# grahamstockton87/RayTracingOneWeekendApplication

Hardware: NVIDIA B200
Metric: path-tracing throughput (higher is better)
Workload: dtype f32

## Files before the change

raytracingoneweekendapplication_b200/csrc/rt_b200.cu:

```cuda
#include <cuda_runtime.h>

#include <chrono>
#include <cmath>
#include <cstdarg>
#include <cstdio>
#include <cstdlib>
#include <cstring>
#include <string>
#include <thread>
#include <vector>

#include "bvh_build.h"
#include "bvh_wide.h"
#include "prim_derive.h"
#include "bvh_device.cuh"
#include "rt_b200.h"
#include "rt_device.cuh"
#include "rt_wide.cuh"
#ifdef RT_B200_ALT_KERNELS
#include "rt_wavefront.cuh"
#endif

using namespace rtdev;

struct RenderArgs {
    int width, height;
    int max_depth;
    int spp_begin;
    int n_local_samples;
    int sample_stride, sample_offset;
    int seg_len;
    int n_segments;
    int tiles_x, tiles_y, tile_size;
    int tile_stride, tile_offset;
    int n_local_tiles;
    int blocks_per_tile_x, blocks_per_tile_y;
    unsigned long long n_items;
    uint32_t k0, k1;
    int compact;
    int nee_emitters;
    int shadow_point_lights;
};

constexpr float kAccumScale = 268435456.0f;
constexpr float kSampleClamp = 1048576.0f;

#ifdef RT_B200_ALT_KERNELS
#include "rt_kernel_v1.cuh"
#endif

#ifndef RT_TRAV_THRESHOLD
#define RT_TRAV_THRESHOLD 4
#endif
#ifndef RT_B200_DEFAULT_BVH_WIDTH
#define RT_B200_DEFAULT_BVH_WIDTH 2
#endif
#ifndef RT_MIN_BLOCKS
#define RT_MIN_BLOCKS 4
#endif
#ifndef RT_WIDE_MIN_BLOCKS
#define RT_WIDE_MIN_BLOCKS RT_MIN_BLOCKS
#endif
#ifndef RT_V2_THREADS
#define RT_V2_THREADS 256
#endif
constexpr int kTravHistBins = 208;
constexpr int kTravThreshold = RT_TRAV_THRESHOLD;
enum : int { LANE_IDLE = 0, LANE_TRAVERSE = 1, LANE_SHADE = 2 };

template <int WIDTH>
struct TravSel { using Trav = TravW<WIDTH>; using RayConst = RayConstW; };
template <>
struct TravSel<2> { using Trav = rtdev::Trav; using RayConst = rtdev::RayConst; };

enum : int { FEAT_MEDIA = 1, FEAT_MEDIA_GENERAL = 2, FEAT_SPECULAR = 4, FEAT_MSPHERE = 8, FEAT_TRI = 16, FEAT_LIGHTS = 32,
             FEAT_DEFOCUS = 64, FEAT_ALL = 127 };
template <bool STATS, bool LITE, bool NEE = false, int WIDTH = 2, int FEAT = FEAT_ALL>
__global__ void __launch_bounds__(RT_V2_THREADS, WIDTH == 2 ? RT_MIN_BLOCKS : RT_WIDE_MIN_BLOCKS) render_kernel_v2(const __grid_constant__ DevScene S, const __grid_constant__ RenderArgs A,
                                                        unsigned long long* __restrict__ accum,
                                                        unsigned long long* __restrict__ counters, Stats* __restrict__ gstats) {
    constexpr bool NO_TRI = LITE || !(FEAT & FEAT_TRI), NO_DEFOCUS = LITE || !(FEAT & FEAT_DEFOCUS), LIGHTS = !LITE && (FEAT & FEAT_LIGHTS);
    const unsigned lane = threadIdx.x & 31u;
    const unsigned lt_mask = (1u << lane) - 1u;
    Stats st;
    if (STATS) memset(&st, 0, sizeof st);

    unsigned pool_pos = 0, pool_size = 0;
    int blk_x0 = 0, blk_y0 = 0, seg_s0 = 0;
    __shared__ uint32_t lane_slot[RT_V2_THREADS];
    unsigned slot_base = 0;
    bool exhausted = A.max_depth <= 0;

    int state = LANE_IDLE;
    Rng rng;
    rng.pixel = rng.sample = 0;
    rng.k0 = A.k0;
    rng.k1 = A.k1;
    Ray ray;
    ray.o = ray.d = v3(0, 0, 0);
    ray.time = 0;
    V3 L = v3(0, 0, 0), T = v3(1, 1, 1);
    uint32_t bounce = 0, origin_prim = PRIM_NONE;
    float nee_pdf = 0.0f;
    typename TravSel<WIDTH>::Trav tr;
    StackEntry stack_mem[WIDTH == 2 ? STACK_SIZE : 1];
    extern __shared__ uint2 wide_stack_mem[];
    auto stack = [&]() {
        if constexpr (WIDTH == 2) return &stack_mem[0];
        else return SmemStack<RT_V2_THREADS>::make(wide_stack_mem);
    }();
    tr.clear();
    tr.hit.t = 0;
    tr.hit.prim = PRIM_NONE;
    tr.hit.u = tr.hit.v = 0;
    const float kInf = __int_as_float(0x7f800000);
    unsigned seg_steps = 0, n_leaf = 0;
    unsigned long long* hist = reinterpret_cast<unsigned long long*>(gstats + 1);

    while (true) {
        unsigned needy = __ballot_sync(0xffffffffu, state == LANE_IDLE);
        while (needy && !exhausted) {
            if (pool_pos >= pool_size) {
                unsigned long long item = 0;
                if (lane == 0) item = atomicAdd(&counters[0], 1ull);
                item = __shfl_sync(0xffffffffu, item, 0);
                if (item >= A.n_items) {
                    exhausted = true;
                    break;
                }
                const unsigned seg = (unsigned)(item % (unsigned long long)A.n_segments);
                const unsigned long long blk = item / (unsigned long long)A.n_segments;
                const unsigned blocks_per_tile = (unsigned)(A.blocks_per_tile_x * A.blocks_per_tile_y);
                const unsigned local_tile = (unsigned)(blk / blocks_per_tile), in_tile = (unsigned)(blk % blocks_per_tile);
                const unsigned tile = A.tile_offset + local_tile * A.tile_stride;
                blk_x0 = (int)(tile % A.tiles_x) * A.tile_size + (int)(in_tile % A.blocks_per_tile_x) * 8;
                blk_y0 = (int)(tile / A.tiles_x) * A.tile_size + (int)(in_tile / A.blocks_per_tile_x) * 4;
                seg_s0 = (int)seg * A.seg_len;
                pool_size = 32u * (unsigned)min(A.seg_len, A.n_local_samples - seg_s0);
                pool_pos = 0;
                slot_base = (local_tile * (unsigned)A.tile_size + (in_tile / (unsigned)A.blocks_per_tile_x) * 4u) * (unsigned)A.tile_size +
                            (in_tile % (unsigned)A.blocks_per_tile_x) * 8u;
            }
            const unsigned e = pool_pos + __popc(needy & lt_mask);
            if (state == LANE_IDLE && e < pool_size) {
                const int px = blk_x0 + (int)(e & 7u), py = blk_y0 + (int)((e >> 3) & 3u);
                if (px < A.width && py < A.height) {
                    rng.pixel = (uint32_t)(py * A.width + px);
                    rng.sample = (uint32_t)(A.spp_begin + A.sample_offset + (seg_s0 + (int)(e >> 5)) * A.sample_stride);
                    if (A.compact) lane_slot[threadIdx.x] = slot_base + ((e >> 3) & 3u) * (unsigned)A.tile_size + (e & 7u);
                    ray = camera_ray<NO_DEFOCUS>(S, px, py, rng);
                    L = v3(0, 0, 0);
                    T = v3(1, 1, 1);
                    bounce = 0;
                    origin_prim = PRIM_NONE;
                    nee_pdf = 0.0f;
                    tr.init(S, kInf);
                    state = tr.done() ? LANE_SHADE : LANE_TRAVERSE;
                    if (STATS) { st.samples++; st.rays++; seg_steps = n_leaf = 0; }
                }
            }
            pool_pos += min((unsigned)__popc(needy), pool_size - pool_pos);
            needy = __ballot_sync(0xffffffffu, state == LANE_IDLE);
        }
        if (__ballot_sync(0xffffffffu, state != LANE_IDLE) == 0u) break;

        {
            typename TravSel<WIDTH>::RayConst rc;
            rc.set(ray);
            while (true) {
                while (true) {
                    const bool descending = tr.wants_node();
                    if (!STATS) {
                        if (!__any_sync(0xffffffffu, descending)) break;
                    }
                    const unsigned dmask = STATS ? __ballot_sync(0xffffffffu, descending) : 1u;
                    if (dmask == 0u) break;
                    if (STATS) {
                        const unsigned tmask = __ballot_sync(0xffffffffu, state == LANE_TRAVERSE);
                        if (lane == 0) { st.desc_iters++; st.desc_lanes += __popc(dmask); st.desc_trav_lanes += __popc(tmask); }
                    }
                    if (descending) {
                        tr.template node_step<STATS>(S, ray, rc, 0.001f, stack, &st);
                        if (STATS) {
                            seg_steps++;
                            if (tr.done()) {
                                atomicAdd(hist + 128 + min(seg_steps, 63u), 1ull);
                                atomicAdd(hist + 192 + min(n_leaf, 15u), 1ull);
                            }
                        }
                    }
                }
                if (STATS) {
                    const unsigned lmask = __ballot_sync(0xffffffffu, state == LANE_TRAVERSE && !tr.wants_node() && !tr.done());
                    if (lane == 0 && lmask) { st.leaf_iters++; st.leaf_lanes += __popc(lmask); }
                }
                if (state == LANE_TRAVERSE && !tr.wants_node()) {
                    if (!tr.done()) {
                        tr.template leaf_step<STATS, NO_TRI, (FEAT & FEAT_MSPHERE) != 0>(S, ray, rc, 0.001f, origin_prim, stack, &st);
                        if (STATS) {
                            atomicAdd(hist + (n_leaf ? 64 : 0) + min(seg_steps, 63u), 1ull);
                            n_leaf++;
                            seg_steps = 0;
                            if (tr.done()) {
                                atomicAdd(hist + 128, 1ull);
                                atomicAdd(hist + 192 + min(n_leaf, 15u), 1ull);
                            }
                        }
                    }
                    if (tr.done()) state = LANE_SHADE;
                }
                const unsigned active = __ballot_sync(0xffffffffu, state == LANE_TRAVERSE);
                if (active == 0u || __popc(active) < kTravThreshold) break;
            }
        }

        if (STATS) {
            const unsigned smask = __ballot_sync(0xffffffffu, state == LANE_SHADE);
            if (lane == 0) { st.shade_iters++; st.shade_lanes += __popc(smask); }
        }
        if (state == LANE_SHADE) {
            Hit hit = tr.hit;
            int medium = -1;
            if ((FEAT & FEAT_MEDIA) && S.n_media > 0) medium = media_hit<STATS, (FEAT & FEAT_MEDIA_GENERAL) != 0>(S, ray, 0.001f, hit.t, rng, bounce, &st);
            bool done = false;
            if (medium < 0 && hit.prim == PRIM_NONE) {
                L = L + T * v3(S.background);
                done = true;
            } else {
                Surface sf;
                if (medium >= 0) {
                    const DevMedium& md = S.media[medium];
                    sf.t = hit.t;
                    sf.p = fma3(hit.t, ray.d, ray.o);
                    sf.normal = v3(md.normal);
                    sf.front = true;
                    sf.u = sf.v = 0.0f;
                    sf.material = md.material;
                    sf.prim_id = -1;
                    sf.nee_light = 0;
                    origin_prim = PRIM_NONE;
                } else {
                    complete_hit<NO_TRI, (FEAT & FEAT_MSPHERE) != 0>(S, ray, hit, sf, false);
                    origin_prim = hit.prim;
                }
                const DevMaterial& m = S.mats[sf.material];
                float4 u4 = make_float4(0, 0, 0, 0);
                if (m.type != RT_MAT_DIFFUSE_LIGHT && m.type != RT_MAT_EMISSIVE_LIGHT) u4 = rng.draw(bounce, RS_SCATTER);
                V3 att, emitted;
                Ray next;
                const bool scattered = shade_surface<(FEAT & FEAT_SPECULAR) != 0>(S, m, ray, sf, u4, emitted, att, next);
                if (NEE && nee_pdf > 0.0f && medium < 0 && sf.nee_light > 0) {
                    const float d2 = dot(ray.d, ray.d);
                    const float cos_y = fabsf(dot(ray.d, v3(S.nee_lights[sf.nee_light - 1].n))) * rsqrtf(d2);
                    const float p_light = light_density(S, sf.t * sf.t * d2, fmaxf(cos_y, 1e-20f));
                    emitted = (nee_pdf / (nee_pdf + p_light)) * emitted;
                }
                L = L + T * emitted;
                if (!scattered) {
                    done = true;
                } else {
                    if (LIGHTS && S.n_lights > 0) {
                        if (NEE && A.shadow_point_lights) L = L + T * att * point_lighting_shadowed<WIDTH>(S, sf.p, sf.normal, origin_prim, ray.time);
                        else L = L + T * att * point_lighting(S, sf.p, sf.normal);
                    }
                    if (NEE) {
                        nee_pdf = 0.0f;
                        if (A.nee_emitters && S.n_nee_lights > 0 && (m.type == RT_MAT_LAMBERTIAN || m.type == RT_MAT_ISOTROPIC)) {
                            const bool iso = m.type == RT_MAT_ISOTROPIC;
                            nee_pdf = scatter_density(normalize(next.d), sf.normal, iso);
                            L = L + T * att * nee_direct<WIDTH>(S, sf.p, sf.normal, iso, origin_prim, ray.time, rng.draw(bounce, RS_NEE));
                        }
                    }
                    T = T * att;
                    ray = next;
                    bounce++;
                    if (bounce >= (uint32_t)A.max_depth) done = true;
                }
            }
            if (done) {
                unsigned long long* a = accum + 4ull * (A.compact ? lane_slot[threadIdx.x] : rng.pixel);
                if (isfinite(L.x) && isfinite(L.y) && isfinite(L.z)) {
                    atomicAdd(a + 0, __float2ull_rn(fminf(fmaxf(L.x, 0.0f), kSampleClamp) * kAccumScale));
                    atomicAdd(a + 1, __float2ull_rn(fminf(fmaxf(L.y, 0.0f), kSampleClamp) * kAccumScale));
                    atomicAdd(a + 2, __float2ull_rn(fminf(fmaxf(L.z, 0.0f), kSampleClamp) * kAccumScale));
                } else {
                    atomicAdd(a + 3, 1ull);
                    if (STATS) st.nonfinite++;
                }
                state = LANE_IDLE;
            } else {
                tr.init(S, kInf);
                state = tr.done() ? LANE_SHADE : LANE_TRAVERSE;
                if (STATS) { st.rays++; seg_steps = n_leaf = 0; }
            }
        }
    }
    if (STATS) {
        unsigned long long* g = reinterpret_cast<unsigned long long*>(gstats);
        const unsigned long long* l = reinterpret_cast<const unsigned long long*>(&st);
        for (unsigned i = 0; i < sizeof(Stats) / 8; i++) {
            unsigned long long v = l[i];
            for (int off = 16; off > 0; off >>= 1) v += __shfl_down_sync(0xffffffffu, v, off);
            if (lane == 0 && v) atomicAdd(g + i, v);
        }
    }
}

#ifdef RT_B200_ALT_KERNELS
#include "rt_kernel_v3.cuh"
#endif

typedef void (*RenderKernel)(const DevScene, const RenderArgs, unsigned long long*, unsigned long long*, Stats*);
struct FeatInstance {
    bool lite;
    int feat;
    RenderKernel kernel;
};
#define RT_INSTANCE(lite, feat) {lite, feat, render_kernel_v2<false, lite, false, 2, (feat)>}
static const FeatInstance kInstances[] = {
    RT_INSTANCE(true, 0),
    RT_INSTANCE(true, FEAT_MEDIA | FEAT_MSPHERE),
    RT_INSTANCE(true, FEAT_MEDIA | FEAT_MEDIA_GENERAL),
    RT_INSTANCE(false, FEAT_DEFOCUS),
    RT_INSTANCE(false, FEAT_TRI | FEAT_LIGHTS),
};
#undef RT_INSTANCE
constexpr int kNumInstances = (int)(sizeof(kInstances) / sizeof(kInstances[0]));

__device__ __forceinline__ void traverse_uploaded(const DevScene& S, const Ray& ray, float tmin, float tmax, Hit& hit) {
    if (S.wide_width == 8) traverse_sel<8>(S, ray, tmin, tmax, PRIM_NONE, hit);
    else if (S.wide_width == 4) traverse_sel<4>(S, ray, tmin, tmax, PRIM_NONE, hit);
    else traverse_sel<2>(S, ray, tmin, tmax, PRIM_NONE, hit);
}

__host__ __device__ inline void pair_node(float4* n) {
    const float4 a = n[0], b = n[1], c = n[2], e = n[3];
    n[0] = make_float4(a.x, c.x, a.y, c.y);
    n[1] = make_float4(a.z, c.z, b.x, e.x);
    n[2] = make_float4(b.y, e.y, b.z, e.z);
    n[3] = make_float4(a.w, b.w, 0.0f, 0.0f);
}
__global__ void pair_nodes_kernel(float4* __restrict__ nodes, int n) {
    const int i = blockIdx.x * blockDim.x + threadIdx.x;
    if (i < n) pair_node(nodes + 4 * (size_t)i);
}

struct CameraD {
    double center[3], dir00[3], du[3], dv[3];
};

__global__ void aov_kernel(const __grid_constant__ DevScene S, const __grid_constant__ CameraD C, int width, int height,
                           int* __restrict__ prim_id, float* __restrict__ t_out, float* __restrict__ normal, float* __restrict__ point,
                           float* __restrict__ uv) {
    int i = blockIdx.x * blockDim.x + threadIdx.x, j = blockIdx.y * blockDim.y + threadIdx.y;
    if (i >= width || j >= height) return;
    RayD rd;
    for (int k = 0; k < 3; k++) {
        rd.o[k] = C.center[k];
        rd.d[k] = C.dir00[k] + (double)i * C.du[k] + (double)j * C.dv[k];
    }
    rd.time = 0.0;
    Ray ray;
    ray.o = v3((float)rd.o[0], (float)rd.o[1], (float)rd.o[2]);
    ray.d = v3((float)rd.d[0], (float)rd.d[1], (float)rd.d[2]);
    ray.time = 0.0f;
    Hit hit;
    traverse_uploaded(S, ray, 0.001f, __int_as_float(0x7f800000), hit);
    size_t px = (size_t)j * width + i;
    Surface sf;
    sf.prim_id = -1;
    sf.p = sf.normal = v3(0, 0, 0);
    sf.u = sf.v = 0;
    float t = 0.0f;
    if (hit.prim != PRIM_NONE) {
        complete_hit_fp64(S, rd, hit, sf);
        t = sf.t;
    }
    if (prim_id) prim_id[px] = sf.prim_id;
    if (t_out) t_out[px] = t;
    if (normal) { normal[3 * px] = sf.normal.x; normal[3 * px + 1] = sf.normal.y; normal[3 * px + 2] = sf.normal.z; }
    if (point) { point[3 * px] = sf.p.x; point[3 * px + 1] = sf.p.y; point[3 * px + 2] = sf.p.z; }
    if (uv) { uv[2 * px] = sf.u; uv[2 * px + 1] = sf.v; }
}

__global__ void resolve_kernel(const unsigned long long* __restrict__ accum, int n_pixels, double inv_scale_spp,
                               float* __restrict__ rgb_linear, unsigned char* __restrict__ rgb8) {
    int px = blockIdx.x * blockDim.x + threadIdx.x;
    if (px >= n_pixels) return;
    for (int c = 0; c < 3; c++) {
        float lin = (float)((double)accum[4ull * px + c] * inv_scale_spp);
        if (rgb_linear) rgb_linear[3ull * px + c] = lin;
        if (rgb8) {
            float g = lin > 0.0f ? sqrtf(lin) : 0.0f;
            g = fminf(fmaxf(g, 0.0f), 0.999f);
            rgb8[3ull * px + c] = (unsigned char)(int)(255.999f * g);
        }
    }
}

__global__ void probe_texture_kernel(const __grid_constant__ DevScene S, int tex, int n, const float* __restrict__ uvp,
                                     float* __restrict__ rgb) {
    int i = blockIdx.x * blockDim.x + threadIdx.x;
    if (i >= n) return;
    V3 c = tex_value(S, tex, uvp[5 * i], uvp[5 * i + 1], v3(uvp + 5 * i + 2));
    rgb[3 * i] = c.x; rgb[3 * i + 1] = c.y; rgb[3 * i + 2] = c.z;
}

__global__ void probe_scatter_kernel(const __grid_constant__ DevScene S, int mat, int n, const float* __restrict__ in,
                                     const float* __restrict__ uni, float* __restrict__ out) {
    int i = blockIdx.x * blockDim.x + threadIdx.x;
    if (i >= n) return;
    const float* r = in + 16 * (size_t)i;
    Ray ray;
    ray.o = v3(r); ray.d = v3(r + 3); ray.time = r[6];
    Surface sf;
    sf.p = v3(r + 7); sf.normal = v3(r + 10); sf.front = r[13] != 0.0f; sf.u = r[14]; sf.v = r[15];
    sf.material = mat; sf.prim_id = -1;
    const DevMaterial& m = S.mats[mat];
    V3 em = mat_emitted(S, m, sf);
    float4 u4 = make_float4(uni[4 * i], uni[4 * i + 1], uni[4 * i + 2], uni[4 * i + 3]);
    V3 att = v3(0, 0, 0);
    Ray next;
    next.o = next.d = v3(0, 0, 0);
    next.time = 0;
    bool ok = mat_scatter(S, m, ray, sf, u4, att, next);
    float* o = out + 16 * (size_t)i;
    o[0] = ok ? 1.0f : 0.0f;
    o[1] = att.x; o[2] = att.y; o[3] = att.z;
    o[4] = next.o.x; o[5] = next.o.y; o[6] = next.o.z;
    o[7] = next.d.x; o[8] = next.d.y; o[9] = next.d.z;
    o[10] = em.x; o[11] = em.y; o[12] = em.z;
    o[13] = next.time; o[14] = o[15] = 0.0f;
}

__global__ void probe_hit_kernel(const __grid_constant__ DevScene S, int n, const float* __restrict__ rays, int* __restrict__ prim_id,
                                 float* __restrict__ t_out, float* __restrict__ normal, float* __restrict__ uv) {
    int i = blockIdx.x * blockDim.x + threadIdx.x;
    if (i >= n) return;
    const float* r = rays + 9 * (size_t)i;
    Ray ray;
    ray.o = v3(r); ray.d = v3(r + 3); ray.time = r[6];
    Hit hit;
    traverse_uploaded(S, ray, r[7], r[8], hit);
    Surface sf;
    sf.prim_id = -1;
    sf.normal = v3(0, 0, 0);
    sf.u = sf.v = 0;
    sf.t = 0.0f;
    if (hit.prim != PRIM_NONE) complete_hit(S, ray, hit, sf, true);
    if (prim_id) prim_id[i] = sf.prim_id;
    if (t_out) t_out[i] = sf.t;
    if (normal) { normal[3 * i] = sf.normal.x; normal[3 * i + 1] = sf.normal.y; normal[3 * i + 2] = sf.normal.z; }
    if (uv) { uv[2 * i] = sf.u; uv[2 * i + 1] = sf.v; }
}

__global__ void fma_peak_kernel(float* out, int iters, float a, float b) {
// ... 1305 lines not shown
            } else {
                rtwf::wf_extend<false><<<grid_e, 256, 0, stream>>>(ctx->scene, P, ctx->dstats);
                rtwf::wf_shade<false><<<grid_s, 256, 0, stream>>>(ctx->scene, W, P, ctx->accum, ctx->dstats);
            }
            launches += 3;
        }
        CU(ctx, cudaGetLastError());
        CU(ctx, cudaMemcpyAsync(h, P.ctr, sizeof h, cudaMemcpyDeviceToHost, stream));
        CU(ctx, cudaStreamSynchronize(stream));
        if (h[3] == 0) break;
    }
    ctx->stats.kernel_launches = launches;
    return RT_OK;
}
#endif

template <int WIDTH>
static RenderKernel v2_instance(int variant) {
    switch (variant) {
        case 1: return render_kernel_v2<false, true, false, WIDTH>;
        case 2: return render_kernel_v2<true, false, false, WIDTH>;
        default: return render_kernel_v2<false, false, false, WIDTH>;
    }
}
static int v2_effective_width(int variant, int width) { return variant >= 3 ? 2 : width; }
static RenderKernel v2_kernel(int variant, int width) {
    if (variant == 3) return render_kernel_v2<false, true, true, 2>;
    if (variant == 4) return render_kernel_v2<false, false, true, 2>;
    if (variant >= 5 && variant < 5 + kNumInstances) return kInstances[variant - 5].kernel;
    return width == 8 ? v2_instance<8>(variant) : (width == 4 ? v2_instance<4>(variant) : v2_instance<2>(variant));
}
static size_t v2_smem(const DevCtx* ctx, int width) { return width <= 2 ? 0 : (size_t)std::max(ctx->wide_depth, 1) * RT_V2_THREADS * sizeof(uint2); }

static int v2_blocks_per_sm(DevCtx* ctx, int variant, int width, int* out) {
    width = v2_effective_width(variant, width);
    RenderKernel k = v2_kernel(variant, width);
    const size_t smem = v2_smem(ctx, width);
    if (smem) {
        const int pct = (int)std::min<size_t>(100, (100 * RT_WIDE_MIN_BLOCKS * (smem + 1024) + 233471) / 233472);
        CU(ctx, cudaFuncSetAttribute((const void*)k, cudaFuncAttributePreferredSharedMemoryCarveout, pct));
    }
    CU(ctx, cudaOccupancyMaxActiveBlocksPerMultiprocessor(out, (const void*)k, RT_V2_THREADS, smem));
    return RT_OK;
}

static int launch_v2(DevCtx* ctx, int variant, int width, int grid, const RenderArgs& A, cudaStream_t stream, unsigned long long* counters = nullptr) {
    if (!counters) counters = ctx->counters;
    width = v2_effective_width(variant, width);
    v2_kernel(variant, width)<<<grid, RT_V2_THREADS, v2_smem(ctx, width), stream>>>(ctx->scene, A, ctx->accum, counters, ctx->dstats);
    return RT_OK;
}

static int dev_render(DevCtx* ctx, const rt_render_params* p) {
    if (!ctx) return RT_ERR_INVALID;
    if (!p || p->struct_size != sizeof(rt_render_params)) return fail(ctx, RT_ERR_INVALID, "rt_render: bad params struct");
    if (!ctx->has_scene) return fail(ctx, RT_ERR_STATE, "rt_render: no scene uploaded");
    if (p->width <= 0 || p->height <= 0 || p->samples_per_pixel <= 0 || p->max_depth < 0 || p->spp_begin < 0)
        return fail(ctx, RT_ERR_INVALID, "rt_render: width/height/samples must be positive");
    if ((long long)p->spp_begin + p->samples_per_pixel > 65536)
        return fail(ctx, RT_ERR_UNSUPPORTED, "rt_render: samples %d + %d exceed 65536 per pixel, the capacity of the 64-bit fixed-point sums",
                    p->spp_begin, p->samples_per_pixel);
    if ((long long)p->width * p->height >= (1ll << 31)) return fail(ctx, RT_ERR_UNSUPPORTED, "rt_render: frame too large");
    const int count = p->shard_count <= 1 ? 1 : p->shard_count;
    const int rank = count == 1 ? 0 : p->shard_rank;
    if (rank < 0 || rank >= count) return fail(ctx, RT_ERR_INVALID, "rt_render: shard_rank %d outside [0,%d)", rank, count);
    CU(ctx, cudaSetDevice(ctx->device));
    cudaStream_t stream = p->stream ? (cudaStream_t)p->stream : ctx->stream;
    const bool overlap = (p->flags & RT_FLAG_OVERLAP) && (p->flags & RT_FLAG_ASYNC) && (p->flags & RT_FLAG_ACCUMULATE) &&
                         !(p->flags & RT_FLAG_STATS) && ctx->kernel_version == 2 && ctx->accum != nullptr &&
                         ctx->cam_w == p->width && ctx->cam_h == p->height;
    int rc = overlap ? RT_OK : dev_wait(ctx);
    if (rc != RT_OK) return rc;
    if (ctx->cam_w != p->width || ctx->cam_h != p->height) setup_camera(ctx, p->width, p->height);

    RenderArgs A;
    std::memset(&A, 0, sizeof A);
    A.width = p->width;
    A.height = p->height;
    A.max_depth = p->max_depth;
    A.spp_begin = p->spp_begin;
    A.tile_size = p->tile_size > 0 ? p->tile_size : 16;
    if (A.tile_size % 8 != 0) return fail(ctx, RT_ERR_INVALID, "rt_render: tile_size must be a multiple of 8");
    A.tiles_x = (p->width + A.tile_size - 1) / A.tile_size;
    A.tiles_y = (p->height + A.tile_size - 1) / A.tile_size;
    A.blocks_per_tile_x = A.tile_size / 8;
    A.blocks_per_tile_y = A.tile_size / 4;
    const int n_tiles = A.tiles_x * A.tiles_y;
    int mode = p->shard_mode;
    if (mode == RT_SHARD_AUTO) mode = (n_tiles / count >= 256) ? RT_SHARD_TILES : RT_SHARD_SAMPLES;
    if (count == 1) mode = RT_SHARD_TILES;
    if (mode == RT_SHARD_TILES) {
        A.tile_stride = count;
        A.tile_offset = rank;
        A.n_local_tiles = (n_tiles - rank + count - 1) / count;
        A.sample_stride = 1;
        A.sample_offset = 0;
        A.n_local_samples = p->samples_per_pixel;
    } else if (mode == RT_SHARD_SAMPLES) {
        A.tile_stride = 1;
        A.tile_offset = 0;
        A.n_local_tiles = n_tiles;
        A.sample_stride = count;
        A.sample_offset = rank;
        A.n_local_samples = (p->samples_per_pixel - rank + count - 1) / count;
    } else {
        return fail(ctx, RT_ERR_INVALID, "rt_render: unknown shard_mode %d", p->shard_mode);
    }
    AccumLayout L;
    L.width = p->width;
    L.height = p->height;
    if (p->flags & RT_FLAG_COMPACT_TILES) {
        if (mode != RT_SHARD_TILES) return fail(ctx, RT_ERR_INVALID, "rt_render: RT_FLAG_COMPACT_TILES needs tile sharding (shard_mode RT_SHARD_TILES)");
        if (ctx->kernel_version != 2) return fail(ctx, RT_ERR_UNSUPPORTED, "rt_render: compact tile buffers are implemented by render_kernel_v2 only");
        L.compact = true;
        L.rank = rank;
        L.count = count;
        L.tile = A.tile_size;
        A.compact = 1;
    }
    if ((p->flags & RT_FLAG_ACCUMULATE) && ctx->accum && !(ctx->acc == L))
        return fail(ctx, RT_ERR_STATE, "rt_render: RT_FLAG_ACCUMULATE onto a buffer of another frame size or tile layout");
    rc = ensure_accum(ctx, L);
    if (rc != RT_OK) return rc;
    const bool stats = (p->flags & RT_FLAG_STATS) != 0;
    int bps = ctx->blocks_per_sm[stats ? 1 : 0];
    const bool lite = ctx->scene_lite && !getenv("RT_B200_NO_LITE");
    const bool want_nee = (p->flags & RT_FLAG_NEE) != 0 && ctx->scene.n_nee_lights > 0;
    const bool want_shadow = (p->flags & RT_FLAG_SHADOWED_POINT_LIGHTS) != 0 && ctx->scene.n_lights > 0;
    int variant = (want_nee || want_shadow) ? (lite ? 3 : 4) : (stats ? 2 : (lite ? 1 : 0));
    const int width = ctx->scene.wide_width ? ctx->scene.wide_width : 2;
    if (variant <= 1 && width == 2 && !getenv("RT_B200_GENERAL_INSTANCE"))
        for (int k = 0; k < kNumInstances; k++)
            if ((!kInstances[k].lite || lite) && (ctx->scene_feat & ~kInstances[k].feat) == 0) {
                variant = 5 + k;
                break;
            }
    if (ctx->kernel_version == 2) {
        rc = v2_blocks_per_sm(ctx, variant, width, &bps);
        if (rc != RT_OK) return rc;
    }
    const int grid = ctx->sm_count * (bps > 0 ? bps : 1);
    const unsigned long long pixel_blocks = (unsigned long long)A.n_local_tiles * A.blocks_per_tile_x * A.blocks_per_tile_y;
    const unsigned long long resident_warps = (unsigned long long)grid * (ctx->kernel_version == 2 ? RT_V2_THREADS / 32 : 8);
    int n_seg = 1;
    if (A.n_local_samples > 0 && pixel_blocks > 0) {
        unsigned long long want = (resident_warps * 64 + pixel_blocks - 1) / pixel_blocks;
        if (want < 1) want = 1;
        if (want > (unsigned long long)A.n_local_samples) want = A.n_local_samples;
        n_seg = (int)want;
    }
    A.seg_len = A.n_local_samples > 0 ? (A.n_local_samples + n_seg - 1) / n_seg : 1;
    A.n_segments = A.n_local_samples > 0 ? (A.n_local_samples + A.seg_len - 1) / A.seg_len : 0;
    A.n_items = pixel_blocks * (unsigned long long)A.n_segments;
    A.k0 = (uint32_t)(p->seed & 0xffffffffu);
    A.k1 = (uint32_t)(p->seed >> 32);

    auto pass_samples = [&]() -> uint64_t {
        if (!(mode == RT_SHARD_TILES && count > 1)) return (uint64_t)A.n_local_samples * (uint64_t)p->width * p->height;
        uint64_t px = 0;
        for (int t = rank; t < n_tiles; t += count) {
            int tx = t % A.tiles_x, ty = t / A.tiles_x;
            int w = std::min(A.tile_size, p->width - tx * A.tile_size), h = std::min(A.tile_size, p->height - ty * A.tile_size);
            px += (uint64_t)w * h;
        }
        return px * (uint64_t)A.n_local_samples;
    };
    if (overlap) {
        const int k = ctx->lane_next;
        ctx->lane_next ^= 1;
        if (!ctx->lane_stream[k]) {
            CU(ctx, cudaStreamCreateWithFlags(&ctx->lane_stream[k], cudaStreamNonBlocking));
            CU(ctx, cudaEventCreateWithFlags(&ctx->lane_end[k], cudaEventDefault));
        }
        if (!ctx->ev_fork) {
            CU(ctx, cudaEventCreateWithFlags(&ctx->ev_fork, cudaEventDisableTiming));
            CU(ctx, cudaEventCreate(&ctx->ov_begin));
        }
        cudaStream_t ls = ctx->lane_stream[k];
        unsigned long long* cnt = ctx->counters + 4 * (1 + k);
        CU(ctx, cudaEventRecord(ctx->ev_fork, stream));
        CU(ctx, cudaStreamWaitEvent(ls, ctx->ev_fork, 0));
        if (!ctx->lane_busy[0] && !ctx->lane_busy[1]) {
            CU(ctx, cudaEventRecord(ctx->ov_begin, ls));
            ctx->ov_passes = 0;
        }
        CU(ctx, cudaMemsetAsync(cnt, 0, 4 * sizeof(unsigned long long), ls));
        if (A.n_items > 0) {
            A.nee_emitters = want_nee;
            A.shadow_point_lights = want_shadow;
            rc = launch_v2(ctx, variant, width, grid, A, ls, cnt);
            if (rc != RT_OK) return rc;
            CU(ctx, cudaGetLastError());
        }
        CU(ctx, cudaEventRecord(ctx->lane_end[k], ls));
        ctx->lane_busy[k] = true;
        ctx->ov_passes++;
        ctx->stats.kernel_launches = A.n_items > 0 ? 1 : 0;
        ctx->stats.blocks = grid;
        ctx->stats.samples = pass_samples();
        return RT_OK;
    }
    if (!(p->flags & RT_FLAG_ACCUMULATE)) CU(ctx, cudaMemsetAsync(ctx->accum, 0, L.slots() * 32, stream));
    CU(ctx, cudaMemsetAsync(ctx->counters, 0, 4 * sizeof(unsigned long long), stream));
    if (stats) CU(ctx, cudaMemsetAsync(ctx->dstats, 0, sizeof(Stats) + kTravHistBins * sizeof(unsigned long long), stream));
    const bool async = (p->flags & RT_FLAG_ASYNC) != 0;
    CU(ctx, cudaEventRecord(ctx->ev0, stream));
    ctx->stats.kernel_launches = 0;
    if (A.n_items > 0) {
#ifdef RT_B200_ALT_KERNELS
        if (ctx->kernel_version == 3) {
            rc = launch_wavefront(ctx, A, stream, stats, pixel_blocks);
            if (rc != RT_OK) return rc;
        } else if (ctx->kernel_version == 1) {
            if (stats) render_kernel<true><<<grid, 256, 0, stream>>>(ctx->scene, A, ctx->accum, ctx->counters, ctx->dstats);
            else render_kernel<false><<<grid, 256, 0, stream>>>(ctx->scene, A, ctx->accum, ctx->counters, ctx->dstats);
        } else if (ctx->kernel_version == 4) {
            const bool lite = ctx->scene_lite && !getenv("RT_B200_NO_LITE");
            if (stats) render_kernel_v3<true, false><<<grid, 256, 0, stream>>>(ctx->scene, A, ctx->accum, ctx->counters, ctx->dstats);
            else if (lite) render_kernel_v3<false, true><<<grid, 256, 0, stream>>>(ctx->scene, A, ctx->accum, ctx->counters, ctx->dstats);
            else render_kernel_v3<false, false><<<grid, 256, 0, stream>>>(ctx->scene, A, ctx->accum, ctx->counters, ctx->dstats);
        } else
#endif
        {
            A.nee_emitters = want_nee;
            A.shadow_point_lights = want_shadow;
            rc = launch_v2(ctx, variant, width, grid, A, stream);
            if (rc != RT_OK) return rc;
        }
        CU(ctx, cudaGetLastError());
        if (ctx->kernel_version != 3) ctx->stats.kernel_launches = 1;
    }
    ctx->stats.blocks = grid;
    ctx->stats.samples = pass_samples();
    CU(ctx, cudaEventRecord(ctx->ev1, stream));
    ctx->pending_async = true;
    ctx->pending_stats = stats;
    ctx->pending_stream = stream;
    if (async) return RT_OK;
    return dev_wait(ctx);
}

static int dev_resolve_into(DevCtx* ctx, int32_t total_spp, float* dev_lin, unsigned char* dev_rgb8) {
    const size_t n = ctx->acc.slots();
    if (n == 0 || (!dev_lin && !dev_rgb8)) return RT_OK;
    const double inv = 1.0 / ((double)kAccumScale * (double)total_spp);
    resolve_kernel<<<(unsigned)((n + 255) / 256), 256, 0, ctx->stream>>>(ctx->accum, (int)n, inv, dev_lin, dev_rgb8);
    CU(ctx, cudaGetLastError());
    return RT_OK;
}

static int ensure_out(DevCtx* ctx, size_t pixels) {
    if (pixels <= ctx->out_pixels) return RT_OK;
    if (ctx->copy_stream) cudaStreamSynchronize(ctx->copy_stream);
    if (ctx->out_lin) cudaFree(ctx->out_lin);
    if (ctx->out_rgb8) cudaFree(ctx->out_rgb8);
    ctx->out_lin = nullptr;
    ctx->out_rgb8 = nullptr;
    ctx->out_pixels = 0;
    if (cudaMalloc(&ctx->out_lin, pixels * 3 * sizeof(float)) != cudaSuccess || cudaMalloc(&ctx->out_rgb8, pixels * 3) != cudaSuccess)
        return fail(ctx, RT_ERR_NOMEM, "rt_download: cannot allocate the output buffers");
    ctx->out_pixels = pixels;
    return RT_OK;
}

static int dev_resolve_tiles(DevCtx* ctx, int32_t total_spp, float* dev_rgb_linear, uint8_t* dev_rgb8, size_t capacity_pixels) {
    if (!ctx) return RT_ERR_INVALID;
    if (!ctx->accum) return fail(ctx, RT_ERR_STATE, "rt_resolve_tiles: nothing rendered yet");
    if (total_spp <= 0) return fail(ctx, RT_ERR_INVALID, "rt_resolve_tiles: total_spp must be positive");
    if (capacity_pixels < ctx->acc.slots()) return fail(ctx, RT_ERR_INVALID, "rt_resolve_tiles: the buffers hold %zu pixels, the frame has %zu", capacity_pixels, ctx->acc.slots());
    int rc = dev_wait(ctx);
    if (rc != RT_OK) return rc;
    rc = dev_resolve_into(ctx, total_spp, dev_rgb_linear, dev_rgb8);
    if (rc != RT_OK) return rc;
    CU(ctx, cudaStreamSynchronize(ctx->stream));
    return RT_OK;
}

static int dev_untile(DevCtx* ctx, const void* dev_shards, size_t shard_stride_bytes, int32_t bytes_per_pixel, int32_t shard_count, int32_t width,
                      int32_t height, int32_t tile_size, void* host_out) {
    if (!ctx || !dev_shards || !host_out) return RT_ERR_INVALID;
    if (width <= 0 || height <= 0 || tile_size <= 0 || shard_count <= 0 || (bytes_per_pixel != 3 && bytes_per_pixel != 12 && bytes_per_pixel != 32))
        return fail(ctx, RT_ERR_INVALID, "rt_untile: bad arguments");
    CU(ctx, cudaSetDevice(ctx->device));
    const size_t full = (size_t)width * height * bytes_per_pixel;
    int rc = ensure_scratch_out(ctx, full);
    if (rc != RT_OK) return rc;
    CU(ctx, launch_untile(bytes_per_pixel, dev_shards, shard_stride_bytes, shard_count, -1, width, height, tile_size, ctx->frame_scratch, ctx->stream));
    CU(ctx, cudaMemcpyAsync(host_out, ctx->frame_scratch, full, cudaMemcpyDeviceToHost, ctx->stream));
    CU(ctx, cudaStreamSynchronize(ctx->stream));
    return RT_OK;
}

static int frame_slot(DevCtx* ctx, size_t px, bool lin, bool rgb8, DevCtx::OutFrame** out) {
    if (ctx->frames_out >= 2) return fail(ctx, RT_ERR_STATE, "two frames are already outstanding: call rt_frame_end first");
    if (!ctx->copy_stream) CU(ctx, cudaStreamCreateWithFlags(&ctx->copy_stream, cudaStreamNonBlocking));
    if (!ctx->ev_ready) CU(ctx, cudaEventCreateWithFlags(&ctx->ev_ready, cudaEventDisableTiming));
    DevCtx::OutFrame& f = ctx->frames[ctx->frame_head];
    if (!f.done) CU(ctx, cudaEventCreateWithFlags(&f.done, cudaEventDisableTiming));
    const size_t need = (lin ? px * 12 : 0) + 256 + (rgb8 ? px * 3 : 0);
    if (need > f.cap) {
        if (f.pinned) cudaFreeHost(f.pinned);
        f.pinned = nullptr;
        f.cap = 0;
        if (cudaHostAlloc(&f.pinned, need, cudaHostAllocDefault) != cudaSuccess) return fail(ctx, RT_ERR_NOMEM, "cannot allocate %zu bytes of pinned host memory", need);
        f.cap = need;
    }
// ... 270 lines not shown
```

Before: 1855.

## Move per-warp work pool state to shared memory and use fast divisors

Per-warp work-pool bookkeeping (block origin, sample start, pool position, exhausted flag) moves from per-thread registers into a small shared-memory struct that lane 0 updates. The per-thread compact-slot shared array is dropped, and the slot is recomputed at accumulation time with precomputed multiply-shift divisors. The 64-bit div/mod in item decoding is replaced by 32-bit fast division. The aim is lower register pressure and cheaper integer work, at the cost of extra __syncwarp calls and shared-memory reads in the refill loop, plus a new limit on work items.

Measured after the change: 1879 (median of 6 runs). 1.3% higher.

```diff
diff --git a/raytracingoneweekendapplication_b200/csrc/render_args.h b/raytracingoneweekendapplication_b200/csrc/render_args.h
--- /dev/null
+++ b/raytracingoneweekendapplication_b200/csrc/render_args.h
@@ -0,0 +1,86 @@
+#pragma once
+#include <cstdint>
+
+#ifdef __CUDACC__
+#define RT_HDI __host__ __device__ __forceinline__
+#else
+#define RT_HDI inline
+#endif
+
+struct FastDiv {
+    uint32_t mul, shift;
+};
+inline FastDiv make_fast_div(uint32_t d) {
+    uint32_t l = 0;
+    while ((1ull << l) < d) l++;
+    FastDiv f;
+    f.mul = (uint32_t)(((1ull << 32) * ((1ull << l) - d)) / d + 1);
+    f.shift = l;
+    return f;
+}
+RT_HDI uint32_t fast_div(uint32_t n, FastDiv f) {
+#ifdef __CUDA_ARCH__
+    const uint32_t hi = __umulhi(n, f.mul);
+#else
+    const uint32_t hi = (uint32_t)(((uint64_t)n * f.mul) >> 32);
+#endif
+    return (hi + n) >> f.shift;
+}
+
+struct RenderArgs {
+    int width, height;
+    int max_depth;
+    int spp_begin;
+    int n_local_samples;
+    int sample_stride, sample_offset;
+    int seg_len;
+    int n_segments;
+    int tiles_x, tiles_y, tile_size;
+    int tile_stride, tile_offset;
+    int n_local_tiles;
+    int blocks_per_tile_x, blocks_per_tile_y;
+    unsigned long long n_items;
+    uint32_t k0, k1;
+    int compact;
+    int nee_emitters;
+    int shadow_point_lights;
+    FastDiv div_segments, div_tile_blocks, div_tiles_x, div_blocks_x;
+    FastDiv div_width, div_tile_size, div_tile_stride;
+};
+
+inline void set_work_divisors(RenderArgs& A) {
+    A.div_segments = make_fast_div((uint32_t)(A.n_segments > 0 ? A.n_segments : 1));
+    A.div_tile_blocks = make_fast_div((uint32_t)(A.blocks_per_tile_x * A.blocks_per_tile_y));
+    A.div_tiles_x = make_fast_div((uint32_t)A.tiles_x);
+    A.div_blocks_x = make_fast_div((uint32_t)A.blocks_per_tile_x);
+    A.div_width = make_fast_div((uint32_t)A.width);
+    A.div_tile_size = make_fast_div((uint32_t)A.tile_size);
+    A.div_tile_stride = make_fast_div((uint32_t)A.tile_stride);
+}
+
+struct PoolBlock {
+    int x0, y0, s0;
+    uint32_t size;
+};
+RT_HDI PoolBlock pool_block(const RenderArgs& A, uint32_t item) {
+    const uint32_t blk = fast_div(item, A.div_segments), seg = item - blk * (uint32_t)A.n_segments;
+    const uint32_t local_tile = fast_div(blk, A.div_tile_blocks);
+    const uint32_t in_tile = blk - local_tile * (uint32_t)(A.blocks_per_tile_x * A.blocks_per_tile_y);
+    const uint32_t by = fast_div(in_tile, A.div_blocks_x), bx = in_tile - by * (uint32_t)A.blocks_per_tile_x;
+    const uint32_t tile = A.tile_offset + local_tile * A.tile_stride;
+    const uint32_t ty = fast_div(tile, A.div_tiles_x), tx = tile - ty * (uint32_t)A.tiles_x;
+    PoolBlock b;
+    b.x0 = (int)tx * A.tile_size + (int)bx * 8;
+    b.y0 = (int)ty * A.tile_size + (int)by * 4;
+    b.s0 = (int)seg * A.seg_len;
+    b.size = 32u * (uint32_t)(A.seg_len < A.n_local_samples - b.s0 ? A.seg_len : A.n_local_samples - b.s0);
+    return b;
+}
+
+RT_HDI uint32_t compact_slot(const RenderArgs& A, uint32_t pixel) {
+    const uint32_t y = fast_div(pixel, A.div_width), x = pixel - y * (uint32_t)A.width;
+    const uint32_t ty = fast_div(y, A.div_tile_size), tx = fast_div(x, A.div_tile_size);
+    const uint32_t tile = ty * (uint32_t)A.tiles_x + tx;
+    const uint32_t local_tile = fast_div(tile - (uint32_t)A.tile_offset, A.div_tile_stride);
+    return (local_tile * (uint32_t)A.tile_size + (y - ty * (uint32_t)A.tile_size)) * (uint32_t)A.tile_size + (x - tx * (uint32_t)A.tile_size);
+}
diff --git a/raytracingoneweekendapplication_b200/csrc/rt_b200.cu b/raytracingoneweekendapplication_b200/csrc/rt_b200.cu
--- a/raytracingoneweekendapplication_b200/csrc/rt_b200.cu
+++ b/raytracingoneweekendapplication_b200/csrc/rt_b200.cu
@@ -14,6 +14,7 @@
 #include "bvh_wide.h"
 #include "prim_derive.h"
 #include "bvh_device.cuh"
+#include "render_args.h"
 #include "rt_b200.h"
 #include "rt_device.cuh"
 #include "rt_wide.cuh"
@@ -22,25 +23,6 @@
 #endif
 
 using namespace rtdev;
-
-struct RenderArgs {
-    int width, height;
-    int max_depth;
-    int spp_begin;
-    int n_local_samples;
-    int sample_stride, sample_offset;
-    int seg_len;
-    int n_segments;
-    int tiles_x, tiles_y, tile_size;
-    int tile_stride, tile_offset;
-    int n_local_tiles;
-    int blocks_per_tile_x, blocks_per_tile_y;
-    unsigned long long n_items;
-    uint32_t k0, k1;
-    int compact;
-    int nee_emitters;
-    int shadow_point_lights;
-};
 
 constexpr float kAccumScale = 268435456.0f;
 constexpr float kSampleClamp = 1048576.0f;
@@ -75,21 +57,34 @@
 
 enum : int { FEAT_MEDIA = 1, FEAT_MEDIA_GENERAL = 2, FEAT_SPECULAR = 4, FEAT_MSPHERE = 8, FEAT_TRI = 16, FEAT_LIGHTS = 32,
              FEAT_DEFOCUS = 64, FEAT_ALL = 127 };
+__device__ __forceinline__ unsigned lane_id() { return threadIdx.x & 31u; }
+__device__ __forceinline__ unsigned lanemask_lt() {
+    unsigned m;
+    asm("mov.u32 %0, %%lanemask_lt;" : "=r"(m));
+    return m;
+}
 template <bool STATS, bool LITE, bool NEE = false, int WIDTH = 2, int FEAT = FEAT_ALL>
 __global__ void __launch_bounds__(RT_V2_THREADS, WIDTH == 2 ? RT_MIN_BLOCKS : RT_WIDE_MIN_BLOCKS) render_kernel_v2(const __grid_constant__ DevScene S, const __grid_constant__ RenderArgs A,
                                                         unsigned long long* __restrict__ accum,
                                                         unsigned long long* __restrict__ counters, Stats* __restrict__ gstats) {
     constexpr bool NO_TRI = LITE || !(FEAT & FEAT_TRI), NO_DEFOCUS = LITE || !(FEAT & FEAT_DEFOCUS), LIGHTS = !LITE && (FEAT & FEAT_LIGHTS);
-    const unsigned lane = threadIdx.x & 31u;
-    const unsigned lt_mask = (1u << lane) - 1u;
     Stats st;
     if (STATS) memset(&st, 0, sizeof st);
 
-    unsigned pool_pos = 0, pool_size = 0;
-    int blk_x0 = 0, blk_y0 = 0, seg_s0 = 0;
-    __shared__ uint32_t lane_slot[RT_V2_THREADS];
-    unsigned slot_base = 0;
-    bool exhausted = A.max_depth <= 0;
+    struct WarpPool {
+        PoolBlock blk;
+        uint32_t pos;
+        uint32_t dry;
+    };
+    __shared__ WarpPool warp_pool[RT_V2_THREADS / 32];
+    static_assert(sizeof(warp_pool) <= 1024, "render_kernel_v2: static shared memory beyond 1 KB per block costs a block per SM");
+    if (lane_id() == 0) {
+        WarpPool& P = warp_pool[threadIdx.x / 32];
+        P.blk.size = 0;
+        P.pos = 0;
+        P.dry = A.max_depth <= 0;
+    }
+    __syncwarp();
 
     int state = LANE_IDLE;
     Rng rng;
@@ -119,35 +114,29 @@
 
     while (true) {
         unsigned needy = __ballot_sync(0xffffffffu, state == LANE_IDLE);
-        while (needy && !exhausted) {
-            if (pool_pos >= pool_size) {
-                unsigned long long item = 0;
-                if (lane == 0) item = atomicAdd(&counters[0], 1ull);
-                item = __shfl_sync(0xffffffffu, item, 0);
-                if (item >= A.n_items) {
-                    exhausted = true;
-                    break;
+        WarpPool& P = warp_pool[threadIdx.x / 32];
+        while (needy && !P.dry) {
+            if (P.pos >= P.blk.size) {
+                __syncwarp();
+                if (lane_id() == 0) {
+                    const unsigned long long item = atomicAdd(&counters[0], 1ull);
+                    if (item >= A.n_items) {
+                        P.dry = 1;
+                    } else {
+                        P.blk = pool_block(A, (uint32_t)item);
+                        P.pos = 0;
+                    }
                 }
-                const unsigned seg = (unsigned)(item % (unsigned long long)A.n_segments);
-                const unsigned long long blk = item / (unsigned long long)A.n_segments;
-                const unsigned blocks_per_tile = (unsigned)(A.blocks_per_tile_x * A.blocks_per_tile_y);
-                const unsigned local_tile = (unsigned)(blk / blocks_per_tile), in_tile = (unsigned)(blk % blocks_per_tile);
-                const unsigned tile = A.tile_offset + local_tile * A.tile_stride;
-                blk_x0 = (int)(tile % A.tiles_x) * A.tile_size + (int)(in_tile % A.blocks_per_tile_x) * 8;
-                blk_y0 = (int)(tile / A.tiles_x) * A.tile_size + (int)(in_tile / A.blocks_per_tile_x) * 4;
-                seg_s0 = (int)seg * A.seg_len;
-                pool_size = 32u * (unsigned)min(A.seg_len, A.n_local_samples - seg_s0);
-                pool_pos = 0;
-                slot_base = (local_tile * (unsigned)A.tile_size + (in_tile / (unsigned)A.blocks_per_tile_x) * 4u) * (unsigned)A.tile_size +
-                            (in_tile % (unsigned)A.blocks_per_tile_x) * 8u;
+                __syncwarp();
+                if (P.dry) break;
             }
-            const unsigned e = pool_pos + __popc(needy & lt_mask);
-            if (state == LANE_IDLE && e < pool_size) {
-                const int px = blk_x0 + (int)(e & 7u), py = blk_y0 + (int)((e >> 3) & 3u);
+            const unsigned pos = P.pos, size = P.blk.size;
+            const unsigned e = pos + __popc(needy & lanemask_lt());
+            if (state == LANE_IDLE && e < size) {
+                const int px = P.blk.x0 + (int)(e & 7u), py = P.blk.y0 + (int)((e >> 3) & 3u);
                 if (px < A.width && py < A.height) {
                     rng.pixel = (uint32_t)(py * A.width + px);
-                    rng.sample = (uint32_t)(A.spp_begin + A.sample_offset + (seg_s0 + (int)(e >> 5)) * A.sample_stride);
-                    if (A.compact) lane_slot[threadIdx.x] = slot_base + ((e >> 3) & 3u) * (unsigned)A.tile_size + (e & 7u);
+                    rng.sample = (uint32_t)(A.spp_begin + A.sample_offset + (P.blk.s0 + (int)(e >> 5)) * A.sample_stride);
                     ray = camera_ray<NO_DEFOCUS>(S, px, py, rng);
                     L = v3(0, 0, 0);
                     T = v3(1, 1, 1);
@@ -159,7 +148,9 @@
                     if (STATS) { st.samples++; st.rays++; seg_steps = n_leaf = 0; }
                 }
             }
-            pool_pos += min((unsigned)__popc(needy), pool_size - pool_pos);
+            __syncwarp();
+            if (lane_id() == 0) P.pos = pos + min((unsigned)__popc(needy), size - pos);
+            __syncwarp();
             needy = __ballot_sync(0xffffffffu, state == LANE_IDLE);
         }
         if (__ballot_sync(0xffffffffu, state != LANE_IDLE) == 0u) break;
@@ -177,7 +168,7 @@
                     if (dmask == 0u) break;
                     if (STATS) {
                         const unsigned tmask = __ballot_sync(0xffffffffu, state == LANE_TRAVERSE);
-                        if (lane == 0) { st.desc_iters++; st.desc_lanes += __popc(dmask); st.desc_trav_lanes += __popc(tmask); }
+                        if (lane_id() == 0) { st.desc_iters++; st.desc_lanes += __popc(dmask); st.desc_trav_lanes += __popc(tmask); }
                     }
                     if (descending) {
                         tr.template node_step<STATS>(S, ray, rc, 0.001f, stack, &st);
@@ -192,7 +183,7 @@
                 }
                 if (STATS) {
                     const unsigned lmask = __ballot_sync(0xffffffffu, state == LANE_TRAVERSE && !tr.wants_node() && !tr.done());
-                    if (lane == 0 && lmask) { st.leaf_iters++; st.leaf_lanes += __popc(lmask); }
+                    if (lane_id() == 0 && lmask) { st.leaf_iters++; st.leaf_lanes += __popc(lmask); }
                 }
                 if (state == LANE_TRAVERSE && !tr.wants_node()) {
                     if (!tr.done()) {
@@ -216,7 +207,7 @@
 
         if (STATS) {
             const unsigned smask = __ballot_sync(0xffffffffu, state == LANE_SHADE);
-            if (lane == 0) { st.shade_iters++; st.shade_lanes += __popc(smask); }
+            if (lane_id() == 0) { st.shade_iters++; st.shade_lanes += __popc(smask); }
         }
         if (state == LANE_SHADE) {
             Hit hit = tr.hit;
@@ -278,7 +269,7 @@
                 }
             }
             if (done) {
-                unsigned long long* a = accum + 4ull * (A.compact ? lane_slot[threadIdx.x] : rng.pixel);
+                unsigned long long* a = accum + 4ull * (A.compact ? compact_slot(A, rng.pixel) : rng.pixel);
                 if (isfinite(L.x) && isfinite(L.y) && isfinite(L.z)) {
                     atomicAdd(a + 0, __float2ull_rn(fminf(fmaxf(L.x, 0.0f), kSampleClamp) * kAccumScale));
                     atomicAdd(a + 1, __float2ull_rn(fminf(fmaxf(L.y, 0.0f), kSampleClamp) * kAccumScale));
@@ -301,7 +292,7 @@
         for (unsigned i = 0; i < sizeof(Stats) / 8; i++) {
             unsigned long long v = l[i];
             for (int off = 16; off > 0; off >>= 1) v += __shfl_down_sync(0xffffffffu, v, off);
-            if (lane == 0 && v) atomicAdd(g + i, v);
+            if (lane_id() == 0 && v) atomicAdd(g + i, v);
         }
     }
 }
@@ -1913,6 +1904,9 @@
     A.seg_len = A.n_local_samples > 0 ? (A.n_local_samples + n_seg - 1) / n_seg : 1;
     A.n_segments = A.n_local_samples > 0 ? (A.n_local_samples + A.seg_len - 1) / A.seg_len : 0;
     A.n_items = pixel_blocks * (unsigned long long)A.n_segments;
+    if (A.n_items >= (1ull << 31))
+        return fail(ctx, RT_ERR_UNSUPPORTED, "rt_render: %llu work items (tile_size %d) exceed 2^31", A.n_items, A.tile_size);
+    set_work_divisors(A);
     A.k0 = (uint32_t)(p->seed & 0xffffffffu);
     A.k1 = (uint32_t)(p->seed >> 32);
 
```
